# AssafSinger94/dino-tracker

Hardware: AMD Instinct MI355X
Metric: query-points*frames/s (higher is better)
Workload: dtype mixed: fp16 ViT operands (one per value), f16 conv operands in Delta-DINO, f16 candidates + f32 deciders in the tracker; f32 accumulate; 1 GPU; 854x480x90 synthetic video (model res 854x476, 67x121 tokens, C=384), 1024 grid queries; 1 video(s) per step over 1 GPU(s); features=vit, mode=single, track_method=mfma, anchor_pairs=92091, correlation_maps_per_video=8380350, rccl_ranks=1, parallelism=video-parallel x1

## Files before the change

dino_tracker_amd/_lib.py:

```python
from __future__ import annotations

import ctypes
import os

_HERE = os.path.dirname(os.path.abspath(__file__))
LIB_PATH = os.path.join(_HERE, "csrc", "libdtk.so")

c_int, c_float, c_void_p, c_size_t = ctypes.c_int, ctypes.c_float, ctypes.c_void_p, ctypes.c_size_t


class Geom(ctypes.Structure):
    _fields_ = [("T", ctypes.c_int32), ("C", ctypes.c_int32), ("ph", ctypes.c_int32), ("pw", ctypes.c_int32),
                ("video_h", ctypes.c_int32), ("video_w", ctypes.c_int32), ("patch", ctypes.c_int32),
                ("stride", ctypes.c_int32), ("radius", ctypes.c_float)]

    @property
    def HW(self) -> int:
        return self.ph * self.pw


def make_geom(T: int, C: int, video_h: int, video_w: int, patch: int = 14, stride: int = 7, radius: float = 35.0) -> Geom:
    ph = 1 + (video_h - patch) // stride
    pw = 1 + (video_w - patch) // stride
    return Geom(T, C, ph, pw, video_h, video_w, patch, stride, radius)
# ... 62 lines not shown
                [(n, ctypes.c_int64) for n in ("in_stride", "in2_stride", "out_stride", "res_stride", "mul_stride", "gate_stride")])


class RaftModel(ctypes.Structure):
    _fields_ = [("conv", RaftConvDesc * RAFT_NUM_CONVS)]


class TrackStats(ctypes.Structure):
    _fields_ = [("sources", ctypes.c_int32), ("whole_map_tier", ctypes.c_int32), ("exact_tier", ctypes.c_int32),
                ("syncs", ctypes.c_int32)]

    def as_dict(self):
        return {k: int(getattr(self, k)) for k, _ in self._fields_}


SIGNATURES = {
    "dtk_version": (c_int, []),
    "dtk_last_error": (ctypes.c_char_p, []),
    "dtk_profile_enable": (c_int, [c_int]),
    "dtk_profile_collect": (c_int, []),
    "dtk_profile_name": (ctypes.c_char_p, [c_int]),
    "dtk_profile_ms": (ctypes.c_double, [c_int]),
    "dtk_profile_launches": (ctypes.c_longlong, [c_int]),
    "dtk_pack_features": (c_int, [c_void_p, c_void_p, c_void_p, c_int, c_int, c_int, c_void_p]),
    "dtk_unpack_features": (c_int, [c_void_p, c_void_p, c_int, c_int, c_int, c_void_p]),
    "dtk_feature_norms": (c_int, [c_void_p, c_void_p, c_int, c_int, c_int, c_void_p]),
    "dtk_vit_workspace_bytes": (c_size_t, [ctypes.POINTER(VitModel), c_int, c_int, c_int]),
    "dtk_vit_forward": (c_int, [ctypes.POINTER(VitModel), c_void_p, c_int, c_int, c_int, c_void_p, c_void_p, c_void_p,
                                c_void_p, c_size_t, c_void_p]),
    "dtk_vit_attention": (c_int, [c_void_p, c_void_p, c_void_p, c_void_p, c_int, c_int, c_int, c_int, c_int, c_void_p]),
    "dtk_vit_attention_split": (c_int, [c_void_p] * 8 + [c_int, c_int, c_int, c_int, c_int, c_void_p]),
    "dtk_vit_gemm": (c_int, [ctypes.POINTER(VitGemmArgs), c_void_p]),
    "dtk_vit_gemm_split": (c_int, [ctypes.POINTER(VitGemmArgs), c_void_p]),
    "dtk_delta_dino_packed_floats": (c_size_t, [c_int, c_int]),
    "dtk_delta_dino_pack": (c_int, [c_int, c_int, c_void_p, c_void_p, c_void_p, c_void_p, c_void_p, c_void_p, c_float,
                                    c_void_p, c_void_p]),
    "dtk_delta_dino_workspace_bytes": (c_size_t, [ctypes.POINTER(Geom)]),
    "dtk_delta_dino_refine": (c_int, [ctypes.POINTER(Geom), c_void_p, c_void_p, ctypes.POINTER(c_void_p), c_void_p,
                                      c_void_p, c_int, c_int, c_void_p, c_size_t, c_void_p]),
    "dtk_delta_dino_refine_mode": (c_int, [ctypes.POINTER(Geom), c_void_p, c_void_p, ctypes.POINTER(c_void_p), c_void_p,
                                           c_void_p, c_int, c_int, c_int, c_void_p, c_size_t, c_void_p]),
    "dtk_sample_points": (c_int, [ctypes.POINTER(Geom), c_void_p, c_void_p, c_void_p, c_void_p, c_void_p, c_int, c_void_p]),
    "dtk_sample_grid": (c_int, [c_void_p, c_int, c_int, c_int, c_int, c_void_p, c_void_p, c_int, c_void_p]),
    "dtk_normalized_conv2d": (c_int, [c_void_p, c_void_p, c_void_p, c_void_p, c_int, c_int, c_int, c_int, c_int, c_int,
                                      c_void_p]),
    "dtk_corr_maps": (c_int, [ctypes.POINTER(Geom), c_void_p, c_void_p, c_void_p, c_void_p, c_void_p, c_void_p, c_void_p,
                              c_int, c_int, c_void_p]),
    "dtk_head_prepare": (c_int, [c_void_p, c_void_p, c_void_p, c_void_p, c_void_p, c_void_p]),
    "dtk_head_forward": (c_int, [ctypes.POINTER(Geom), c_void_p, c_void_p, c_void_p, c_int, c_int, c_void_p]),
    "dtk_head_forward_train": (c_int, [ctypes.POINTER(Geom), c_void_p, c_void_p, c_void_p, c_void_p, c_int, c_int, c_void_p]),
    "dtk_conv_split_weight_halves": (c_size_t, [c_int, c_int]),
    "dtk_conv_split_pack": (c_int, [c_void_p, c_int, c_int, c_int, c_void_p, c_void_p, c_void_p]),
    "dtk_conv_split_input": (c_int, [c_void_p, c_int, c_int, c_int, c_int, c_int, c_void_p, c_void_p, c_void_p, c_void_p]),
    "dtk_conv_split_run": (c_int, [c_void_p, c_void_p, c_void_p, c_void_p, c_void_p, c_int, c_int, c_int, c_int, c_int, c_int,
                                   c_int, c_int, c_void_p]),
    "dtk_conv_split_output": (c_int, [c_void_p, c_int, c_int, c_int, c_int, c_int, c_int, c_void_p, c_void_p, c_void_p]),
    "dtk_conv_wgrad_split_workspace_bytes": (c_size_t, [c_int, c_int, c_int, c_int, c_int, c_int]),
    "dtk_conv_wgrad_split": (c_int, [c_void_p, c_void_p, c_void_p, c_int, c_int, c_int, c_int, c_int, c_int, c_int, c_void_p,
                                     c_int, c_void_p, c_size_t, c_void_p]),
    "dtk_gemm_nt_f32_indexed": (c_int, [c_void_p, c_void_p, c_void_p, c_int, c_int, c_int, ctypes.c_int64, ctypes.c_int64,
                                        ctypes.c_int64, c_int, ctypes.c_int64, ctypes.c_int64, ctypes.c_int64, c_int, c_int,
                                        c_void_p, c_void_p, c_void_p, c_void_p, c_void_p]),
    "dtk_contrastive_workspace_bytes": (c_size_t, [c_int, c_int, c_int, c_int]),
    "dtk_contrastive_forward": (c_int, [c_void_p, c_void_p, c_void_p, ctypes.c_float, c_int, c_int, c_int, c_int, c_int, c_void_p,
                                        c_void_p, c_void_p, c_void_p, c_void_p, c_void_p]),
    "dtk_contrastive_backward": (c_int, [c_void_p, c_void_p, c_void_p, ctypes.c_float, c_int, c_int, c_int, c_int, c_int, c_void_p,
# ... 150 lines not shown
```

dino_tracker_amd/csrc/vit.hip:

```cpp
#include <stdlib.h>
#include "common.h"
#include "vit_attention4.h"
#include "vit_attention6.h"
#include "vit_gemm_common.h"
#include "vit_rowwise.h"
#include "vit_patch_embed.h"
#include "vit_gemm_tiled.h"
#include "vit_gemm_ws.h"
#include "vit_gemm_ws_ln.h"
#include "vit_gemm_wide.h"
#include "vit_split.h"

namespace {

constexpr int VIT_FRAME_BATCH = 90;

struct VitPlan {
    int S, Sp, FB;
    size_t x, xn, q, k, vt, ao, hid, delta, total;
    bool split;
    size_t xn_lo, q_lo, k_lo, vt_lo, ao_lo, hid_lo;
};

inline bool vit_layer_split(const dtk_vit_layer& L) { return L.qkv_w_lo != nullptr; }
// ... 40 lines not shown
    } else {
        const unsigned grid = attn::attention_grid(FH, S, 128 * attn::A6_NQ, &QB);
        DTK_LAUNCH("vit_attention", (attn::attention6_kernel<T, 0>), dim3(grid), dim3(256), 0, st, q, k, vt, o, S, Sp, heads, D,
                   FH, QB);
    }
    return DTK_OK;
}
template <typename T>
int attention_split_launch(const T* q, const T* q_lo, const T* k, const T* k_lo, const T* vt, const T* vt_lo, T* o, T* o_lo, int frames,
                           int heads, int S, int Sp, hipStream_t st) {
    const int nqb = dtk_cdiv(Sp, 128);
    DTK_LAUNCH("vit_attention_split", attention_split_kernel<T>, dim3((unsigned)(frames * heads * nqb)), dim3(256), 0, st, q, q_lo, k, k_lo,
               vt, vt_lo, o, o_lo, S, Sp, heads, nqb);
    return DTK_OK;
}

struct GemmPath {
    bool tiled;
    bool ws;
    bool wide;
    bool ws_v1;
    bool wide_v1;
    bool fc2_ln;
    bool proj_ln;
};
inline GemmPath gemm_path(int D, int f) {
    const bool tiled = (f & DTK_VIT_TILED_GEMMS) != 0, ws = !tiled && D == WS_K, wide_v1 = (f & DTK_VIT_GEMM_WIDE_V1) != 0;
    static_assert(WS_K == WD_N, "fc2 of the weight-stationary width is gemm_wide_delta_kernel's shape");
    const bool ws_v1 = (f & DTK_VIT_GEMM_WS_V1) != 0, fc2_ln = ws && !wide_v1 && !(f & DTK_VIT_NO_LN_FUSION);
    return {tiled, ws, !tiled && D % W2_N == 0, ws_v1, wide_v1, fc2_ln, fc2_ln && !ws_v1};
}
inline GemmPath gemm_path(const dtk_vit_model* m) { return gemm_path(m->D, m->flags); }

template <typename T, int EPI>
int launch_gemm(const char* name, const GemmPath& path, const T* A, const T* W, long long rows, int N, int K, const GemmEpi<T>& e,
                hipStream_t st) {
    if constexpr (EPI != EPI_F32) {
        const bool ws_fits = EPI != EPI_QKV || e.S >= WS_ROWS || rows <= e.S;
        if constexpr (EPI == EPI_DELTA) {
            if (path.ws && K == WS_K && N == WS_K && e.ln_out) {
                const auto gr = gemm_ws_ln_grid(rows);
                DTK_LAUNCH(name, (gemm_ws_ln_kernel<T>), gr.first, dim3(256), 0, st, A, W, rows, e, gr.second);
                return DTK_OK;
            }
        }
        if (path.ws && K == WS_K && ws_fits) {
            const auto gr = gemm_ws_grid(N, rows);
            if (path.ws_v1)
                DTK_LAUNCH(name, (gemm_ws_kernel<T, EPI, 0>), gr.first, dim3(256), 0, st, A, W, rows, N, e, gr.second);
            else if (N % 64 != 0 || DTK_DBG(e.no_store, 128))
                DTK_LAUNCH(name, (gemm_ws_kernel<T, EPI, 3, false>), gr.first, dim3(256), 0, st, A, W, rows, N, e, gr.second);
            else
                DTK_LAUNCH(name, (gemm_ws_kernel<T, EPI>), gr.first, dim3(256), 0, st, A, W, rows, N, e, gr.second);
            return DTK_OK;
        }
        if (path.ws && EPI == EPI_DELTA) {
            const dim3 grid(dtk_cdiv(rows, WD_M));
            if (path.wide_v1)
                DTK_LAUNCH(name, (gemm_wide_delta_kernel<T, false>), grid, dim3(512), 0, st, A, W, rows, K, e);
            else if (e.ln_out)
                DTK_LAUNCH(name, (gemm_wide_delta_kernel<T, true, true>), grid, dim3(512), 0, st, A, W, rows, K, e);
            else
                DTK_LAUNCH(name, (gemm_wide_delta_kernel<T, true>), grid, dim3(512), 0, st, A, W, rows, K, e);
            return DTK_OK;
        }
        if (path.wide) {
            const dim3 grid(gemm_wide_grid(N, rows));
            if (path.wide_v1)
                DTK_LAUNCH(name, (gemm_wide_kernel<T, EPI, false>), grid, dim3(512), 0, st, A, W, rows, N, K, e);
            else
                DTK_LAUNCH(name, (gemm_wide_kernel<T, EPI, true>), grid, dim3(512), 0, st, A, W, rows, N, K, e);
            return DTK_OK;
        }
    }
    DTK_LAUNCH(name, (gemm_tiled_kernel<T, EPI>), dim3(gemm_grid(N, rows)), dim3(256), 0, st, A, W, rows, N, K, e);
// ... 327 lines not shown
                                 int Sp, int operand_type, void* stream) {
    DTK_REQUIRE(q && k && vt && out, "dtk_vit_attention: null pointer");
    DTK_REQUIRE(frames > 0 && heads > 0 && S > 0 && Sp >= S && Sp % 64 == 0, "dtk_vit_attention: bad sizes (Sp %% 64 == 0, Sp >= S)");
    const bool v4 = (operand_type & DTK_OPERAND_ATTENTION_V4) != 0;
    operand_type &= ~DTK_OPERAND_ATTENTION_V4;
    DTK_REQUIRE(operand_type == DTK_OPERAND_F16 || operand_type == DTK_OPERAND_BF16, "dtk_vit_attention: operand_type");
    return with_operand_type(operand_type == DTK_OPERAND_BF16, [&](auto t) {
        typedef decltype(t) T;
        return attention_launch(reinterpret_cast<const T*>(q), reinterpret_cast<const T*>(k), reinterpret_cast<const T*>(vt),
                                reinterpret_cast<T*>(out), S, Sp, heads, heads * VIT_D_HEAD, frames * heads, v4, dtk_stream(stream));
    });
}

extern "C" int dtk_vit_attention_split(const void* q_hi, const void* q_lo, const void* k_hi, const void* k_lo, const void* vt_hi,
                                       const void* vt_lo, void* out_hi, void* out_lo, int frames, int heads, int S, int Sp,
                                       int operand_type, void* stream) {
    DTK_REQUIRE(q_hi && q_lo && k_hi && k_lo && vt_hi && vt_lo && out_hi && out_lo, "dtk_vit_attention_split: null pointer");
    DTK_REQUIRE(frames > 0 && heads > 0 && S > 0 && Sp >= S && Sp % 64 == 0, "dtk_vit_attention_split: bad sizes (Sp %% 64 == 0, Sp >= S)");
    DTK_REQUIRE(operand_type == DTK_OPERAND_F16 || operand_type == DTK_OPERAND_BF16, "dtk_vit_attention_split: operand_type");
    return with_operand_type(operand_type == DTK_OPERAND_BF16, [&](auto t) {
        typedef decltype(t) T;
        return attention_split_launch<T>((const T*)q_hi, (const T*)q_lo, (const T*)k_hi, (const T*)k_lo, (const T*)vt_hi, (const T*)vt_lo,
                                         (T*)out_hi, (T*)out_lo, frames, heads, S, Sp, dtk_stream(stream));
    });
}

extern "C" int dtk_vit_gemm(const dtk_vit_gemm_args* g, void* stream) {
    if (const int rc = vit_gemm_check(g, "dtk_vit_gemm", false)) return rc;
    return with_operand_type(g->operand_type == DTK_OPERAND_BF16, [&](auto t) {
        return run_gemm<decltype(t)>(*g, gemm_path(g->D, g->flags), vit_gemm_hidden(g), dtk_stream(stream));
    });
}

extern "C" int dtk_vit_gemm_split(const dtk_vit_gemm_args* g, void* stream) {
    if (const int rc = vit_gemm_check(g, "dtk_vit_gemm_split", true)) return rc;
    DTK_REQUIRE(!g->ln_out, "dtk_vit_gemm_split: the split blocks have their own LayerNorm");
    return with_operand_type(g->operand_type == DTK_OPERAND_BF16, [&](auto t) {
        return run_gemm_split<decltype(t)>(*g, gemm_path(g->D, g->flags), vit_gemm_hidden(g), dtk_stream(stream));
    });
}
```

dino_tracker_amd/csrc/vit_gemm_ws.h:

```cpp
#pragma once
#include <type_traits>
#include <utility>
#include "vit_gemm_common.h"

namespace {

constexpr int WS_KS = 24, WS_K = 16 * WS_KS, WS_ROWS = 32, WS_COLS = 256;
constexpr int WS_TILE_BYTES = WS_ROWS * WS_K * 2;
constexpr int WS_LQ = WS_KS / 4;
constexpr int WS_PITCH = 144;
constexpr int WS_UNIT_BYTES = WS_ROWS * WS_PITCH;

template <class F, int... I>
__device__ __forceinline__ void ws_for_each(F&& f, std::integer_sequence<int, I...>) { (f(std::integral_constant<int, I>{}), ...); }
template <int N, class F>
__device__ __forceinline__ void ws_for_each(F&& f) { ws_for_each(f, std::make_integer_sequence<int, N>{}); }

template <typename T, int EPI, int V2M = 3, bool HC = (V2M == 3)>
__global__ __launch_bounds__(256) void gemm_ws_kernel(const T* __restrict__ A, const T* __restrict__ Wt,
                                                      long long M, int N, GemmEpi<T> e, int tiles_per_chunk) {
    typedef typename Vec<T>::t8 T8;
    typedef typename Vec<T>::t4 T4;
    (void)sizeof(T8); (void)sizeof(T4);
    constexpr bool V2 = (V2M & 1) != 0;
    constexpr bool V2D = (V2M & 2) != 0;
    static_assert(!HC || V2M == 3, "the hand-cut step is built on the AGPR weights and the descriptor LDS-DMA");
    operand_mode<T>();
    __shared__ __attribute__((aligned(1024))) unsigned char toks[3][WS_TILE_BYTES];
    __shared__ __attribute__((aligned(16))) unsigned char stage[4][2][WS_UNIT_BYTES];
    __shared__ __attribute__((aligned(16))) float s_bias[4][64], s_gamma[4][64];
    const int tid = threadIdx.x, lane = tid & 63;
    const int w = __builtin_amdgcn_readfirstlane(tid >> 6);
    const int j = lane & 31, h = lane >> 5;
    const int n0 = blockIdx.x * WS_COLS + w * 64;
    const long long total_tiles = (M + WS_ROWS - 1) / WS_ROWS;
    const long long tile0 = (long long)blockIdx.y * tiles_per_chunk;
    if (tile0 >= total_tiles) return;
    const int NT = (int)((total_tiles - tile0) < tiles_per_chunk ? (total_tiles - tile0) : tiles_per_chunk);
    const int nl = (j & 3) + 4 * (j >> 3) + 16 * ((j >> 2) & 1);
    T8 wf[2][WS_KS];
#pragma unroll
    for (int t = 0; t < 2; ++t) {
        const int row = min(n0 + t * 32 + nl, N - 1);
        const T* wp = Wt + (size_t)row * WS_K + h * 8;
#pragma unroll
        for (int ks = 0; ks < WS_KS; ++ks) {
            if (V2) asm volatile("global_load_dwordx4 %0, %1, off" : "=a"(wf[t][ks]) : "v"(wp + ks * 16) : "memory");
            else wf[t][ks] = *reinterpret_cast<const T8*>(wp + ks * 16);
        }
    }
    if (V2) {
        asm volatile("s_waitcnt vmcnt(0)" ::: "memory");
#pragma unroll
        for (int t = 0; t < 2; ++t)
#pragma unroll
            for (int ks = 0; ks < WS_KS; ++ks) asm volatile("" : "+a"(wf[t][ks]));
    }
    if constexpr (!HC) {
        const int n = min(n0 + lane, N - 1);
        s_bias[w][lane] = e.bias ? e.bias[n] : 0.f;
        s_gamma[w][lane] = (EPI == EPI_DELTA) ? e.gamma[n] : 1.f;
    }
    const int which = (EPI == EPI_QKV) ? min(n0, N - 1) / e.D : 0;
    const int head = (EPI == EPI_QKV) ? (min(n0, N - 1) - which * e.D) >> 6 : 0;
    const float qsc = (EPI == EPI_QKV && which == 0) ? e.qscale : 1.f;
    long long m_ep = tile0 * WS_ROWS + j;
    int f_ep = 0, s_ep = 0;
    if (EPI == EPI_QKV) { f_ep = (int)(m_ep / e.S); s_ep = (int)(m_ep - (long long)f_ep * e.S); }
    const unsigned lds_base = (unsigned)(size_t)&toks[0][0];
    const int l_tt = lane & 3, l_pp = lane >> 2;
    const dtk_u4 srd = dtk_make_srd(A + tile0 * WS_ROWS * WS_K);
    unsigned a_voff[2], a_voff_last[2];
    const int last_rows = (int)(M - (total_tiles - 1) * WS_ROWS);
#pragma unroll
    for (int gg = 0; gg < 2; ++gg) {
        const int g = 2 * w + gg;
        a_voff[gg] = (unsigned)(((4 * g + l_tt) * WS_K + ((l_pp - g) & 15) * 8) * 2);
        a_voff_last[gg] = (unsigned)((min(4 * g + l_tt, last_rows - 1) * WS_K + ((l_pp - g) & 15) * 8) * 2);
    }
    const unsigned a_dst = __builtin_amdgcn_readfirstlane(lds_base + (2 * w) * 3 * 1024);
    auto issue = [&](int n, int buf) {
        if (V2D) {
            const unsigned toff = __builtin_amdgcn_readfirstlane((unsigned)n * (unsigned)WS_TILE_BYTES);
            const unsigned dst = __builtin_amdgcn_readfirstlane(a_dst + (unsigned)buf * (unsigned)WS_TILE_BYTES);
            const bool last = tile0 + n == total_tiles - 1;
            const unsigned v0 = last ? a_voff_last[0] : a_voff[0], v1 = last ? a_voff_last[1] : a_voff[1];
            dtk_buffer_lds16<0>(srd, toff, v0, dst);
            dtk_buffer_lds16<1024>(srd, toff + 256u, v0, dst);
            dtk_buffer_lds16<2048>(srd, toff + 512u, v0, dst);
// ... 17 lines not shown
    for (int k8 = 0; k8 < 8; ++k8)
        frag_off[k8] = (unsigned)((j >> 2) * 3 * 1024 + ((((2 * k8 + h + (j >> 2)) & 15) * 4 + (j & 3)) * 16));
    float amax = 0.f;
    unsigned dbg_sink = 0;
    auto dbg_fold = [&](const auto& val) {
        unsigned b[sizeof(val) / 4];
        __builtin_memcpy(b, &val, sizeof(val));
#pragma unroll
        for (unsigned i = 0; i < sizeof(val) / 4; ++i) dbg_sink |= b[i];
    };
    if constexpr (HC) {
        typedef std::integral_constant<bool, true> Yes;
        typedef std::integral_constant<bool, false> No;
        if (n0 >= N) {
            issue(0, 0);
            issue(min(1, NT - 1), 1);
            dtk_vm_wait<WS_LQ>();
            __syncthreads();
            int b0 = 0;
            for (int n = 0; n + 1 < NT; n += 2) {
                const int b1 = b0 == 2 ? 0 : b0 + 1, b2 = b1 == 2 ? 0 : b1 + 1;
                issue(min(n + 2, NT - 1), b2);
                dtk_vm_wait<WS_LQ>();
                __syncthreads();
                issue(min(n + 3, NT - 1), b0);
                dtk_vm_wait<WS_LQ>();
                __syncthreads();
                b0 = b2;
            }
            dtk_vm_wait<0>();
            return;
        }
        float bia[2][16], gam[2][16];
#pragma unroll
        for (int t = 0; t < 2; ++t)
#pragma unroll
            for (int r = 0; r < 16; ++r) {
                const int nf = n0 + 32 * t + 16 * h + r;
                bia[t][r] = e.bias ? e.bias[nf] : 0.f;
                gam[t][r] = (EPI == EPI_DELTA) ? e.gamma[nf] : 1.f;
            }
        const bool dbg_nost = DTK_DBG(e.no_store, 3) || DTK_DBG(e.no_store, 32);
        const bool dbg_noar = DTK_DBG(e.no_store, 64);
        auto run = [&](auto vt_tag) {
            constexpr bool VT = decltype(vt_tag)::value;
            constexpr bool STG = EPI != EPI_GELU && !VT;
            const long long mt0 = tile0 * WS_ROWS;
            T* op = nullptr;
            T* up = nullptr;
            int s0 = 0;
            unsigned cross = 0;
            if constexpr (EPI == EPI_GELU) op = e.out + (mt0 + j) * N + n0 + 16 * h;
            if constexpr (EPI == EPI_DELTA) up = e.delta + mt0 * N + n0;
            if constexpr (EPI == EPI_QKV) {
                const int f0 = (int)(mt0 / e.S);
                s0 = (int)(mt0 - (long long)f0 * e.S);
                if (VT) {
                    up = e.vt + (((size_t)f0 * e.heads + head) * 64) * e.Sp + s0;
                    cross = (unsigned)(e.heads * 64 * e.Sp - e.S);
                } else {
                    up = (which == 0 ? e.q : e.k) + (((size_t)f0 * e.heads + head) * e.Sp + s0) * 64;
                    cross = (unsigned)((e.heads * e.Sp - e.S) * 64);
                }
            }
            const size_t out_step = (size_t)WS_ROWS * N;
            unsigned char* const sw = &stage[w][0][0] + j * WS_PITCH + 32 * h;
            const unsigned char* const sr = &stage[w][0][0] + (lane >> 3) * WS_PITCH + (lane & 7) * 16;
            auto next_tile = [&]() {
                if constexpr (EPI == EPI_GELU) op += out_step;
                if constexpr (EPI == EPI_DELTA) up += out_step;
                if constexpr (EPI == EPI_QKV) {
                    s0 += WS_ROWS;
                    up += VT ? WS_ROWS : WS_ROWS * 64;
                    if (s0 >= e.S) { s0 -= e.S; up += cross; }
                }
            };
            auto st16 = [&](T* p, unsigned off, dtk_u4 val, bool ok) {
                if (!dbg_nost) { if (ok) *reinterpret_cast<dtk_u4*>(p + off) = val; }
                else dbg_fold(val);
            };
            float v[8];
            f2 sx[4], uu[4], pp[4];
            T8 o;
            dtk_u4 fv[4];
            unsigned voff = 0;
            constexpr float GC[9] = {1.112979639e-10f, -1.065557687e-08f, 4.510875158e-07f, -1.125288873e-05f, 1.868377149e-04f,
                                     -2.217123518e-03f, 1.963194646e-02f, -1.326889843e-01f, 7.978046536e-01f};
            auto flush_reads = [&]() {
                ws_for_each<4>([&](auto p_tag) {
                    constexpr int p = decltype(p_tag)::value;
                    fv[p] = *reinterpret_cast<const dtk_u4*>(sr + 8 * p * WS_PITCH);
                });
            };
            auto flush_store = [&](auto pred_tag, auto p_tag, int valid) {
                constexpr int p = decltype(p_tag)::value;
                const int row = 8 * p + (lane >> 3);
                const bool ok = decltype(pred_tag)::value ? row < valid : true;
                if constexpr (EPI == EPI_DELTA) st16(up, (unsigned)(row * N + (lane & 7) * 8), fv[p], ok);
                else st16(up, (unsigned)(row * 64 + (lane & 7) * 8) + (s0 + row >= e.S ? cross : 0u), fv[p], ok);
            };
            auto slot = [&](auto pred_tag, auto fl_tag, const f16v (&acc)[2], auto s_tag, int valid) {
                constexpr bool PRED = decltype(pred_tag)::value, FL = decltype(fl_tag)::value;
                constexpr int s = decltype(s_tag)::value;
                const bool ok = PRED ? j < valid : true;
                if constexpr (EPI == EPI_GELU) {
                    constexpr int u = s / 12, ph = s % 12, t = u >> 1, hv = u & 1;
                    if (ph < 2) {
#pragma unroll
                        for (int r = 4 * ph; r < 4 * ph + 4; ++r) v[r] = acc[t][8 * hv + r] + bia[t][8 * hv + r];
                        if (IsF16<T>::value) {
#pragma unroll
                            for (int r = 4 * ph; r < 4 * ph + 4; r += 2) amax = fmaxf(fmaxf(amax, v[r]), v[r + 1]);
                        }
                    }
                    if (dbg_noar) {
                        if (ph == 9) {
#pragma unroll
                            for (int r = 0; r < 8; ++r) o[r] = (T)v[r];
                        }
                    } else if (ph == 2) {
                        const f2 c = {4.25f, 4.25f};
#pragma unroll
                        for (int q = 0; q < 4; ++q) sx[q] = __builtin_elementwise_min(__builtin_elementwise_max(f2{v[2 * q], v[2 * q + 1]}, -c), c);
#pragma unroll
                        for (int q = 0; q < 4; ++q) uu[q] = sx[q] * sx[q];
                    } else if (ph >= 3 && ph <= 6) {
#pragma unroll
                        for (int l = 2 * (ph - 3); l < 2 * (ph - 3) + 2; ++l)
#pragma unroll
                            for (int q = 0; q < 4; ++q)
                                pp[q] = __builtin_elementwise_fma(l == 0 ? f2{GC[0], GC[0]} : pp[q], uu[q], f2{GC[l + 1], GC[l + 1]});
                    } else if (ph == 7) {
                        const f2 one = {1.f, 1.f};
#pragma unroll
                        for (int q = 0; q < 4; ++q) pp[q] = __builtin_elementwise_min(__builtin_elementwise_max(sx[q] * pp[q], -one), one);
                    } else if (ph == 8) {
#pragma unroll
                        for (int q = 0; q < 4; ++q) {
                            const f2 hx = f2{v[2 * q], v[2 * q + 1]} * f2{0.5f, 0.5f};
                            uu[q] = __builtin_elementwise_fma(hx, pp[q], hx);
                        }
                    } else if (ph == 9) {
#pragma unroll
                        for (int q = 0; q < 4; ++q) { o[2 * q] = (T)uu[q][0]; o[2 * q + 1] = (T)uu[q][1]; }
                    }
                    if (ph == 10) {
                        st16(op, (unsigned)(32 * t + 8 * hv), __builtin_bit_cast(dtk_u4, o), ok);
                    }
                } else if constexpr (STG) {
                    if constexpr (FL && s == 0) flush_reads();
                    if constexpr (FL && s >= 1 && s <= 4) flush_store(No{}, std::integral_constant<int, s - 1>{}, WS_ROWS);
                    constexpr int u = s / 12, ph = s % 12, t = u >> 1, hv = u & 1;
                    if (ph & 1) {
                        if (ph < 9) {
                            constexpr int r0 = (ph - 1) & 7, r1 = ph & 7;
                            const float v0 = acc[t][8 * hv + r0] + bia[t][8 * hv + r0], v1 = acc[t][8 * hv + r1] + bia[t][8 * hv + r1];
                            if (EPI == EPI_QKV && IsF16<T>::value && !dbg_noar) amax = amax2(amax, v0 * qsc, v1 * qsc);
                            if (dbg_noar) { o[r0] = (T)v0; o[r1] = (T)v1; }
                            else if (EPI == EPI_DELTA) { o[r0] = (T)(v0 * gam[t][8 * hv + r0]); o[r1] = (T)(v1 * gam[t][8 * hv + r1]); }
                            else { o[r0] = (T)(v0 * qsc); o[r1] = (T)(v1 * qsc); }
                        } else if (ph == 9) {
                            *reinterpret_cast<T8*>(sw + 64 * t + 16 * hv) = o;
                        }
                    }
                } else {
                    if (s == 0) voff = (unsigned)(16 * h * e.Sp + j) + (s0 + j >= e.S ? cross : 0u);
                    if (s < 32) {
                        constexpr int u = (s & 31) / 8, r = s % 8, t = u >> 1, hv = u & 1;
                        v[r] = acc[t][8 * hv + r] + bia[t][8 * hv + r];
                        if (IsF16<T>::value && (r & 1) && !dbg_noar) amax = amax2(amax, v[r - 1] * qsc, v[r] * qsc);
                        const T val = (T)v[r];
                        T* const p = up + (size_t)(32 * t + 8 * hv + r) * e.Sp;
                        if (!dbg_nost) { if (ok) p[voff] = val; }
                        else dbg_fold(typename Vec<T>::t2{val, val});
                    }
                }
            };
            auto tail_epi = [&](const f16v (&acc)[2], int valid) {
                ws_for_each<2 * WS_KS>([&](auto s_tag) { slot(Yes{}, No{}, acc, s_tag, valid); });
                if (!STG) next_tile();
            };
            auto tail_flush = [&](int valid) {
                if constexpr (STG) {
                    flush_reads();
                    ws_for_each<4>([&](auto p_tag) { flush_store(Yes{}, p_tag, valid); });
                    next_tile();
                }
            };
            auto step = [&](auto prev_tag, auto fl_tag, int buf, f16v (&accN)[2], const f16v (&accP)[2]) {
                constexpr bool PREV = decltype(prev_tag)::value, FL = decltype(fl_tag)::value;
                const unsigned char* base = &toks[0][0] + buf * WS_TILE_BYTES;
                const f16v zero16 = {0.f, 0.f, 0.f, 0.f, 0.f, 0.f, 0.f, 0.f, 0.f, 0.f, 0.f, 0.f, 0.f, 0.f, 0.f, 0.f};
                T8 b[3];
                b[0] = *reinterpret_cast<const T8*>(base + frag_off[0]);
                b[1] = *reinterpret_cast<const T8*>(base + frag_off[1]);
                ws_for_each<2 * WS_KS>([&](auto s_tag) {
                    constexpr int ks = decltype(s_tag)::value / 2, t = decltype(s_tag)::value % 2;
                    if constexpr (t == 0 && ks + 2 < WS_KS)
                        b[(ks + 2) % 3] = *reinterpret_cast<const T8*>(base + frag_off[(ks + 2) & 7] + ((ks + 2) >> 3) * 1024);
                    accN[t] = mfma32(wf[t][ks], b[ks % 3], ks == 0 ? zero16 : accN[t]);
                    if constexpr (PREV) {
                        __builtin_amdgcn_sched_barrier(0);
                        slot(No{}, fl_tag, accP, s_tag, WS_ROWS);
                        __builtin_amdgcn_sched_barrier(0);
                    }
                });
                if (STG ? FL : PREV) next_tile();
            };
            f16v accA[2], accB[2];
            issue(0, 0);
            issue(min(1, NT - 1), 1);
            dtk_vm_wait<WS_LQ>();
            __syncthreads();
            int n = 0, b0 = 0;
            auto pair = [&](auto first_tag) {
                constexpr bool FIRST = decltype(first_tag)::value;
                const int b1 = b0 == 2 ? 0 : b0 + 1, b2 = b1 == 2 ? 0 : b1 + 1;
                issue(min(n + 2, NT - 1), b2);
                if (FIRST) step(No{}, No{}, b0, accA, accB);
                else step(Yes{}, Yes{}, b0, accA, accB);
                dtk_vm_wait<WS_LQ>();
                __syncthreads();
                issue(min(n + 3, NT - 1), b0);
                if (FIRST) step(Yes{}, No{}, b1, accB, accA);
                else step(Yes{}, Yes{}, b1, accB, accA);
                dtk_vm_wait<WS_LQ>();
                __syncthreads();
                b0 = b2;
                n += 2;
            };
            if (NT >= 2) pair(Yes{});
            while (n + 1 < NT) pair(No{});
            const long long left = M - (tile0 + NT - 1) * WS_ROWS;
            const int valid = left < WS_ROWS ? (int)left : WS_ROWS;
            const bool odd = n < NT;
            if (odd) {
                if (n > 0) step(Yes{}, Yes{}, b0, accA, accB);
                else step(No{}, No{}, b0, accA, accB);
            }
            if (NT > 1) tail_flush(WS_ROWS);
            const f16v accL[2] = {odd ? accA[0] : accB[0], odd ? accA[1] : accB[1]};
            tail_epi(accL, valid);
            tail_flush(valid);
        };
        if constexpr (EPI == EPI_QKV) {
            if (which == 2) run(Yes{});
            else run(No{});
        } else {
            run(No{});
        }
        if (DTK_DBG(e.no_store, 32) && dbg_sink == 0x9e3779b9u) amax = 65504.f;
        amax_report<T, EPI>(amax, e.ovf);
        dtk_vm_wait<0>();
        return;
    }
    auto epi8 = [&](const f16v (&acc)[2], int t, int hv) {
        const int fl = 32 * t + 16 * h + 8 * hv;
        const int nb = n0 + fl;
        const float4 b0 = *reinterpret_cast<const float4*>(&s_bias[w][fl]), b1 = *reinterpret_cast<const float4*>(&s_bias[w][fl + 4]);
        float v[8];
#pragma unroll
        for (int r = 0; r < 8; ++r) v[r] = acc[t][8 * hv + r];
        v[0] += b0.x; v[1] += b0.y; v[2] += b0.z; v[3] += b0.w;
        v[4] += b1.x; v[5] += b1.y; v[6] += b1.z; v[7] += b1.w;
        const bool ok = m_ep < M && nb < N && !DTK_DBG(e.no_store, 3);
        if (IsF16<T>::value && (EPI == EPI_QKV || EPI == EPI_GELU)) {
#pragma unroll
            for (int r = 0; r < 8; r += 2) {
                if (EPI == EPI_GELU) amax = fmaxf(fmaxf(amax, v[r]), v[r + 1]);
                else if (!DTK_DBG(e.no_store, 64)) amax = amax2(amax, v[r] * qsc, v[r + 1] * qsc);
            }
        }
        if (EPI == EPI_GELU) {
            T8 o;
#pragma unroll
// ... 139 lines not shown
```

include/dtk.h:

```cpp
#ifndef DTK_H_
#define DTK_H_

#include <stddef.h>
#include <stdint.h>

#ifdef __cplusplus
extern "C" {
#endif

#define DTK_OK 0
#define DTK_E_INVALID (-1)
#define DTK_E_HIP (-2)
#define DTK_E_WORKSPACE (-3)

typedef struct dtk_geom {
    int32_t T;
    int32_t C;
    int32_t ph, pw;
    int32_t video_h, video_w;
    int32_t patch, stride;
    float radius;
} dtk_geom;

#define DTK_HEAD_HIDDEN 16
// ... 67 lines not shown
int dtk_vit_forward(const dtk_vit_model* m, const float* frames, int nframes, int video_h, int video_w,
                    float* tokens_out, float* feat_out, float* qkv_out, void* workspace, size_t workspace_bytes,
                    void* stream);

int dtk_vit_attention(const void* q, const void* k, const void* vt, void* out, int frames, int heads, int S, int Sp,
                      int operand_type, void* stream);
int dtk_vit_attention_split(const void* q_hi, const void* q_lo, const void* k_hi, const void* k_lo, const void* vt_hi,
                            const void* vt_lo, void* out_hi, void* out_lo, int frames, int heads, int S, int Sp, int operand_type,
                            void* stream);

#define DTK_VIT_GEMM_QKV 0
#define DTK_VIT_GEMM_QKV_FACET 1
#define DTK_VIT_GEMM_PROJ 2
#define DTK_VIT_GEMM_FC1 3
#define DTK_VIT_GEMM_FC2 4
#define DTK_VIT_GEMM_FC1_SWIGLU 5
#define DTK_VIT_GEMM_FC2_SWIGLU 6
typedef struct dtk_vit_gemm_args {
    int32_t role, D, flags, operand_type;
    int64_t rows;
    int32_t S, Sp;
    float ln_eps, w_scale;
    const void *a, *a_lo, *w, *w_lo;
    const float *bias, *gamma;
    void *q, *k, *vt, *q_lo, *k_lo, *vt_lo;
    void *out, *out_lo;
    float *out_f32, *x, *ln_x;
    const float *ln_w, *ln_b;
    void* ln_out;
    int32_t* ovf;
} dtk_vit_gemm_args;
int dtk_vit_gemm(const dtk_vit_gemm_args* g, void* stream);
int dtk_vit_gemm_split(const dtk_vit_gemm_args* g, void* stream);

size_t dtk_delta_dino_packed_floats(int layer, int C);
int dtk_delta_dino_pack(int layer, int C, const float* w, const float* bias, const float* bn_w, const float* bn_b,
                        const float* bn_mean, const float* bn_var, float eps, float* packed, void* stream);
size_t dtk_delta_dino_workspace_bytes(const dtk_geom* g);
int dtk_delta_dino_refine(const dtk_geom* g, const float* video, const float* dino, const float* const* packed,
                          float* out, float* norms, int t0, int nframes, void* workspace, size_t workspace_bytes,
                          void* stream);
#define DTK_DD_SPLIT 0
#define DTK_DD_FP16 1
#define DTK_DD_FP16_V1 2
int dtk_delta_dino_refine_mode(const dtk_geom* g, const float* video, const float* dino, const float* const* packed,
                               float* out, float* norms, int t0, int nframes, int operands, void* workspace,
                               size_t workspace_bytes, void* stream);

int dtk_sample_points(const dtk_geom* g, const float* feat, const float* xy, const int32_t* t_idx,
                      const int32_t* out_row, float* out, int B, void* stream);

int dtk_sample_grid(const float* feat, int T, int C, int ph, int pw, const float* pts, float* out, int B, void* stream);

int dtk_head_prepare(const float* w1, const float* b1, const float* w2, const float* b2, float* head, void* stream);

int dtk_head_forward(const dtk_geom* g, const float* head, const float* maps, float* out_xy, int B, int normalized,
                     void* stream);

int dtk_head_forward_train(const dtk_geom* g, const float* head, const float* maps, float* out_xy, float* stats, int B,
                           int normalized, void* stream);
int dtk_head_backward(const dtk_geom* g, const float* head, const float* maps, const float* stats, const float* grad_out,
                      float* dmaps, float* dhead_partial, int B, int normalized, void* stream);

size_t dtk_conv_split_weight_halves(int Cin, int Cout);
int dtk_conv_split_pack(const float* w, int Cin, int Cout, int flip_transpose, void* Wh, void* Wl, void* stream);
int dtk_conv_split_input(const float* x, int N, int C, int H, int W, int border, const float* scale, void* hi, void* lo,
// ... 338 lines not shown
```

Baseline: 528,500 query-points*frames/s.

## Widen weight-stationary fc1/qkv GEMM waves to 96 columns with per-group chunk plan

Adds an RT=3 variant of the weight-stationary GEMM in which each wave holds 96 output columns of weights (partly in AGPRs, partly in VGPRs) instead of 64. A workgroup then covers 384 columns, so each streamed token tile is reused across more MFMAs. A new launch plan splits the grid into column groups with their own tiles-per-chunk, giving the V group of qkv a tuned share of workgroups. QKV output is staged through a larger LDS buffer for coalesced stores, and GELU bias now comes from LDS. The risks are higher register pressure, lower occupancy and a more complex epilogue schedule.

```diff
diff --git a/dino_tracker_amd/_lib.py b/dino_tracker_amd/_lib.py
--- a/dino_tracker_amd/_lib.py
+++ b/dino_tracker_amd/_lib.py
@@ -118,6 +118,8 @@
     "dtk_vit_attention_split": (c_int, [c_void_p] * 8 + [c_int, c_int, c_int, c_int, c_int, c_void_p]),
     "dtk_vit_gemm": (c_int, [ctypes.POINTER(VitGemmArgs), c_void_p]),
     "dtk_vit_gemm_split": (c_int, [ctypes.POINTER(VitGemmArgs), c_void_p]),
+    "dtk_vit_gemm_ws_plan": (c_int, [c_int, c_int, c_int, ctypes.c_int64, c_int, ctypes.POINTER(c_int), ctypes.POINTER(c_int),
+                                     ctypes.POINTER(c_int)]),
     "dtk_delta_dino_packed_floats": (c_size_t, [c_int, c_int]),
     "dtk_delta_dino_pack": (c_int, [c_int, c_int, c_void_p, c_void_p, c_void_p, c_void_p, c_void_p, c_void_p, c_float,
                                     c_void_p, c_void_p]),
diff --git a/dino_tracker_amd/csrc/vit.hip b/dino_tracker_amd/csrc/vit.hip
--- a/dino_tracker_amd/csrc/vit.hip
+++ b/dino_tracker_amd/csrc/vit.hip
@@ -96,15 +96,27 @@
 }
 inline GemmPath gemm_path(const dtk_vit_model* m) { return gemm_path(m->D, m->flags); }
 
+inline bool gemm_ws_fits(int epi, long long rows, int S) { return epi != EPI_QKV || S >= WS_ROWS || rows <= S; }
+inline bool gemm_ws96_runs(const GemmPath& path, int epi, long long rows, int N, int K, int S, int no_store) {
+    return gemm_ws96_role(epi) && path.ws && K == WS_K && gemm_ws_fits(epi, rows, S) && !path.ws_v1 && gemm_ws96_fits(N) && !DTK_DBG(no_store, 128);
+}
+
 template <typename T, int EPI>
 int launch_gemm(const char* name, const GemmPath& path, const T* A, const T* W, long long rows, int N, int K, const GemmEpi<T>& e,
                 hipStream_t st) {
     if constexpr (EPI != EPI_F32) {
-        const bool ws_fits = EPI != EPI_QKV || e.S >= WS_ROWS || rows <= e.S;
+        const bool ws_fits = gemm_ws_fits(EPI, rows, e.S);
         if constexpr (EPI == EPI_DELTA) {
             if (path.ws && K == WS_K && N == WS_K && e.ln_out) {
                 const auto gr = gemm_ws_ln_grid(rows);
                 DTK_LAUNCH(name, (gemm_ws_ln_kernel<T>), gr.first, dim3(256), 0, st, A, W, rows, e, gr.second);
+                return DTK_OK;
+            }
+        }
+        if constexpr (gemm_ws96_role(EPI)) {
+            if (gemm_ws96_runs(path, EPI, rows, N, K, e.S, e.no_store)) {
+                const Ws96Plan plan = gemm_ws96_plan(N, rows);
+                DTK_LAUNCH(name, (gemm_ws_kernel<T, EPI, 3, true, 3>), gemm_ws96_grid(plan), dim3(256), 0, st, A, W, rows, N, e, plan);
                 return DTK_OK;
             }
         }
@@ -498,6 +510,20 @@
     });
 }
 
+extern "C" int dtk_vit_gemm_ws_plan(int role, int D, int flags, int64_t rows, int S, int32_t* chunks, int32_t* tpc, int32_t* last) {
+    if (!chunks || !tpc || !last || rows <= 0 || (role != DTK_VIT_GEMM_FC1 && role != DTK_VIT_GEMM_QKV)) return 0;
+    const int epi = role == DTK_VIT_GEMM_FC1 ? EPI_GELU : EPI_QKV, N = role == DTK_VIT_GEMM_FC1 ? 4 * D : 3 * D;
+    if (!gemm_ws96_runs(gemm_path(D, flags), epi, rows, N, D, S, 0)) return 0;
+    const Ws96Plan p = gemm_ws96_plan(N, rows);
+    const long long tiles = dtk_cdiv(rows, WS_ROWS);
+    for (int g = 0; g < p.groups; ++g) {
+        chunks[g] = p.chunks[g];
+        tpc[g] = p.tpc[g];
+        last[g] = (int32_t)(tiles - (long long)(p.chunks[g] - 1) * p.tpc[g]);
+    }
+    return p.groups;
+}
+
 extern "C" int dtk_vit_gemm_split(const dtk_vit_gemm_args* g, void* stream) {
     if (const int rc = vit_gemm_check(g, "dtk_vit_gemm_split", true)) return rc;
     DTK_REQUIRE(!g->ln_out, "dtk_vit_gemm_split: the split blocks have their own LayerNorm");
diff --git a/dino_tracker_amd/csrc/vit_gemm_ws.h b/dino_tracker_amd/csrc/vit_gemm_ws.h
--- a/dino_tracker_amd/csrc/vit_gemm_ws.h
+++ b/dino_tracker_amd/csrc/vit_gemm_ws.h
@@ -16,45 +16,108 @@
 template <int N, class F>
 __device__ __forceinline__ void ws_for_each(F&& f) { ws_for_each(f, std::make_integer_sequence<int, N>{}); }
 
-template <typename T, int EPI, int V2M = 3, bool HC = (V2M == 3)>
+constexpr int WS96_COLS = 384, WS96_MAX_GROUPS = 4, WS96_WGS = 256;
+constexpr int WS96_PITCH = WS96_COLS * 2 + 16;
+constexpr int WS96_STAGE_BYTES = WS_ROWS * WS96_PITCH;
+constexpr int WS96_VT_SHARE = 92;
+constexpr int WS96_MAX_TPC = 65536;
+struct Ws96Plan {
+    int groups;
+    int chunks[WS96_MAX_GROUPS];
+    int tpc[WS96_MAX_GROUPS];
+};
+inline Ws96Plan gemm_ws96_plan(int N, long long rows) {
+    Ws96Plan p = {};
+    p.groups = N / WS96_COLS;
+    const long long tiles = (rows + WS_ROWS - 1) / WS_ROWS;
+    int vt_share = WS96_VT_SHARE;
+#ifdef DTK_WS96_SWEEP
+    if (const char* sv = getenv("DTK_WS96_VT_SHARE")) vt_share = atoi(sv);
+#endif
+    for (int g = 0; g < p.groups; ++g) {
+        const int share = p.groups != 3 ? WS96_WGS / p.groups : g == 2 ? vt_share : (WS96_WGS - vt_share) / 2;
+        long long tpc = (tiles + share - 1) / share;
+        if (tpc < 1) tpc = 1;
+        if (tpc > WS96_MAX_TPC) tpc = WS96_MAX_TPC;
+        p.tpc[g] = (int)tpc;
+        p.chunks[g] = (int)((tiles + tpc - 1) / tpc);
+    }
+    return p;
+}
+constexpr bool gemm_ws96_role(int epi) { return epi == EPI_GELU || epi == EPI_QKV; }
+inline bool gemm_ws96_fits(int N) { return N % WS96_COLS == 0 && N / WS96_COLS >= 1 && N / WS96_COLS <= WS96_MAX_GROUPS; }
+inline dim3 gemm_ws96_grid(const Ws96Plan& p) {
+    unsigned n = 0;
+    for (int g = 0; g < p.groups; ++g) n += (unsigned)p.chunks[g];
+    return dim3(n);
+}
+struct WsWhere {
+    unsigned colgroup;
+    int tpc;
+    unsigned chunk;
+};
+template <int RT> struct WsArg { typedef int type; };
+template <> struct WsArg<3> { typedef Ws96Plan type; };
+__device__ __forceinline__ WsWhere ws_where(int tiles_per_chunk) {
+    return {blockIdx.x, tiles_per_chunk, blockIdx.y};
+}
+__device__ __forceinline__ WsWhere ws_where(const Ws96Plan& plan) {
+    int c = blockIdx.x, g = 0, tpc = plan.tpc[0], first = 0;
+#pragma unroll
+    for (int i = 0; i + 1 < WS96_MAX_GROUPS; ++i) {
+        first += plan.chunks[i];
+        if (i + 1 < plan.groups && (int)blockIdx.x >= first) { g = i + 1; c = (int)blockIdx.x - first; tpc = plan.tpc[i + 1]; }
+    }
+    return {(unsigned)g, tpc, (unsigned)c};
+}
+
+template <typename T, int EPI, int V2M = 3, bool HC = (V2M == 3), int RT = 2>
 __global__ __launch_bounds__(256) void gemm_ws_kernel(const T* __restrict__ A, const T* __restrict__ Wt,
-                                                      long long M, int N, GemmEpi<T> e, int tiles_per_chunk) {
+                                                      long long M, int N, GemmEpi<T> e, typename WsArg<RT>::type where) {
     typedef typename Vec<T>::t8 T8;
     typedef typename Vec<T>::t4 T4;
     (void)sizeof(T8); (void)sizeof(T4);
     constexpr bool V2 = (V2M & 1) != 0;
     constexpr bool V2D = (V2M & 2) != 0;
     static_assert(!HC || V2M == 3, "the hand-cut step is built on the AGPR weights and the descriptor LDS-DMA");
+    static_assert(RT == 2 || (RT == 3 && HC && (EPI == EPI_GELU || EPI == EPI_QKV)), "96 features per wave: the hand-cut fc1 and qkv steps only");
+    constexpr int WCOLS = 32 * RT;
+    constexpr int AGPR_FRAGS = RT == 2 ? 2 * WS_KS : 60;
     operand_mode<T>();
     __shared__ __attribute__((aligned(1024))) unsigned char toks[3][WS_TILE_BYTES];
     __shared__ __attribute__((aligned(16))) unsigned char stage[4][2][WS_UNIT_BYTES];
-    __shared__ __attribute__((aligned(16))) float s_bias[4][64], s_gamma[4][64];
+    constexpr bool STG3 = RT == 3 && EPI == EPI_QKV;
+    __shared__ __attribute__((aligned(16))) unsigned char stage3[STG3 ? 2 : 1][STG3 ? WS96_STAGE_BYTES : 16];
+    __shared__ __attribute__((aligned(16))) float s_bias[4][WCOLS], s_gamma[4][64];
     const int tid = threadIdx.x, lane = tid & 63;
     const int w = __builtin_amdgcn_readfirstlane(tid >> 6);
     const int j = lane & 31, h = lane >> 5;
-    const int n0 = blockIdx.x * WS_COLS + w * 64;
+    const WsWhere wh = ws_where(where);
+    const int tiles_per_chunk = wh.tpc;
+    const int n0 = wh.colgroup * (4 * WCOLS) + w * WCOLS;
     const long long total_tiles = (M + WS_ROWS - 1) / WS_ROWS;
-    const long long tile0 = (long long)blockIdx.y * tiles_per_chunk;
+    const long long tile0 = (long long)wh.chunk * tiles_per_chunk;
     if (tile0 >= total_tiles) return;
     const int NT = (int)((total_tiles - tile0) < tiles_per_chunk ? (total_tiles - tile0) : tiles_per_chunk);
     const int nl = (j & 3) + 4 * (j >> 3) + 16 * ((j >> 2) & 1);
-    T8 wf[2][WS_KS];
-#pragma unroll
-    for (int t = 0; t < 2; ++t) {
+    T8 wf[RT][WS_KS];
+#pragma unroll
+    for (int t = 0; t < RT; ++t) {
         const int row = min(n0 + t * 32 + nl, N - 1);
         const T* wp = Wt + (size_t)row * WS_K + h * 8;
 #pragma unroll
         for (int ks = 0; ks < WS_KS; ++ks) {
-            if (V2) asm volatile("global_load_dwordx4 %0, %1, off" : "=a"(wf[t][ks]) : "v"(wp + ks * 16) : "memory");
+            if (V2 && t * WS_KS + ks < AGPR_FRAGS) asm volatile("global_load_dwordx4 %0, %1, off" : "=a"(wf[t][ks]) : "v"(wp + ks * 16) : "memory");
             else wf[t][ks] = *reinterpret_cast<const T8*>(wp + ks * 16);
         }
     }
     if (V2) {
         asm volatile("s_waitcnt vmcnt(0)" ::: "memory");
 #pragma unroll
-        for (int t = 0; t < 2; ++t)
-#pragma unroll
-            for (int ks = 0; ks < WS_KS; ++ks) asm volatile("" : "+a"(wf[t][ks]));
+        for (int t = 0; t < RT; ++t)
+#pragma unroll
+            for (int ks = 0; ks < WS_KS; ++ks)
+                if (t * WS_KS + ks < AGPR_FRAGS) asm volatile("" : "+a"(wf[t][ks]));
     }
     if constexpr (!HC) {
         const int n = min(n0 + lane, N - 1);
@@ -138,14 +201,19 @@
             return;
         }
         float bia[2][16], gam[2][16];
-#pragma unroll
-        for (int t = 0; t < 2; ++t)
-#pragma unroll
-            for (int r = 0; r < 16; ++r) {
-                const int nf = n0 + 32 * t + 16 * h + r;
-                bia[t][r] = e.bias ? e.bias[nf] : 0.f;
-                gam[t][r] = (EPI == EPI_DELTA) ? e.gamma[nf] : 1.f;
-            }
+        if constexpr (RT == 2) {
+#pragma unroll
+            for (int t = 0; t < 2; ++t)
+#pragma unroll
+                for (int r = 0; r < 16; ++r) {
+                    const int nf = n0 + 32 * t + 16 * h + r;
+                    bia[t][r] = e.bias ? e.bias[nf] : 0.f;
+                    gam[t][r] = (EPI == EPI_DELTA) ? e.gamma[nf] : 1.f;
+                }
+        } else {
+            (void)bia; (void)gam;
+            for (int i = lane; i < WCOLS; i += 64) s_bias[w][i] = e.bias ? e.bias[n0 + i] : 0.f;
+        }
         const bool dbg_nost = DTK_DBG(e.no_store, 3) || DTK_DBG(e.no_store, 32);
         const bool dbg_noar = DTK_DBG(e.no_store, 64);
         auto run = [&](auto vt_tag) {
@@ -168,6 +236,10 @@
                     up = (which == 0 ? e.q : e.k) + (((size_t)f0 * e.heads + head) * e.Sp + s0) * 64;
                     cross = (unsigned)((e.heads * e.Sp - e.S) * 64);
                 }
+                if constexpr (RT == 3) {
+                    if (VT) up = e.vt + ((size_t)f0 * e.heads * 64 + (n0 - which * e.D)) * e.Sp + s0;
+                    else up = (which == 0 ? e.q : e.k) + ((size_t)f0 * e.heads * e.Sp + s0) * 64;
+                }
             }
             const size_t out_step = (size_t)WS_ROWS * N;
             unsigned char* const sw = &stage[w][0][0] + j * WS_PITCH + 32 * h;
@@ -188,28 +260,88 @@
             float v[8];
             f2 sx[4], uu[4], pp[4];
             T8 o;
-            dtk_u4 fv[4];
+            constexpr int NFL = STG3 ? 6 : 4;
+            dtk_u4 fv[NFL];
             unsigned voff = 0;
+            unsigned sto = 0, flo = 0;
+            unsigned char* const sw3 = STG3 ? &stage3[0][0] + j * WS96_PITCH + (w * WCOLS + 16 * h) * 2 : nullptr;
+            const unsigned char* const sr3 = STG3 ? &stage3[0][0] + (tid >> 3) * WS96_PITCH + (lane & 7) * 16 : nullptr;
             constexpr float GC[9] = {1.112979639e-10f, -1.065557687e-08f, 4.510875158e-07f, -1.125288873e-05f, 1.868377149e-04f,
                                      -2.217123518e-03f, 1.963194646e-02f, -1.326889843e-01f, 7.978046536e-01f};
             auto flush_reads = [&]() {
-                ws_for_each<4>([&](auto p_tag) {
+                ws_for_each<NFL>([&](auto p_tag) {
                     constexpr int p = decltype(p_tag)::value;
-                    fv[p] = *reinterpret_cast<const dtk_u4*>(sr + 8 * p * WS_PITCH);
+                    if constexpr (STG3) fv[p] = *reinterpret_cast<const dtk_u4*>(sr3 + flo + 128 * p);
+                    else fv[p] = *reinterpret_cast<const dtk_u4*>(sr + 8 * p * WS_PITCH);
                 });
             };
             auto flush_store = [&](auto pred_tag, auto p_tag, int valid) {
                 constexpr int p = decltype(p_tag)::value;
+                if constexpr (STG3) {
+                    const int row3 = tid >> 3;
+                    const bool ok3 = decltype(pred_tag)::value ? row3 < valid : true;
+                    st16(up, (unsigned)(row3 * 64 + (lane & 7) * 8 + p * e.Sp * 64) + (s0 + row3 >= e.S ? cross : 0u), fv[p], ok3);
+                    return;
+                }
                 const int row = 8 * p + (lane >> 3);
                 const bool ok = decltype(pred_tag)::value ? row < valid : true;
                 if constexpr (EPI == EPI_DELTA) st16(up, (unsigned)(row * N + (lane & 7) * 8), fv[p], ok);
                 else st16(up, (unsigned)(row * 64 + (lane & 7) * 8) + (s0 + row >= e.S ? cross : 0u), fv[p], ok);
             };
-            auto slot = [&](auto pred_tag, auto fl_tag, const f16v (&acc)[2], auto s_tag, int valid) {
+            float4 bi0, bi1, bj0, bj1;
+            auto slot = [&](auto pred_tag, auto fl_tag, const f16v (&acc)[RT], auto s_tag, int valid) {
                 constexpr bool PRED = decltype(pred_tag)::value, FL = decltype(fl_tag)::value;
                 constexpr int s = decltype(s_tag)::value;
                 const bool ok = PRED ? j < valid : true;
-                if constexpr (EPI == EPI_GELU) {
+                if constexpr (EPI == EPI_GELU && RT == 3) {
+                    const float* const sb = &s_bias[w][16 * h];
+                    constexpr int u = s / 12, ph = s % 12, t = u >> 1, hv = u & 1;
+                    if (ph == 0) {
+                        bi0 = *reinterpret_cast<const float4*>(sb + 32 * t + 8 * hv);
+                        bi1 = *reinterpret_cast<const float4*>(sb + 32 * t + 8 * hv + 4);
+                    } else if (ph <= 2) {
+                        const float4 bq = ph == 1 ? bi0 : bi1;
+                        const float bb[4] = {bq.x, bq.y, bq.z, bq.w};
+#pragma unroll
+                        for (int r = 4 * (ph - 1); r < 4 * (ph - 1) + 4; ++r) v[r] = acc[t][8 * hv + r] + bb[r & 3];
+                        if (IsF16<T>::value) {
+#pragma unroll
+                            for (int r = 4 * (ph - 1); r < 4 * (ph - 1) + 4; r += 2) amax = fmaxf(fmaxf(amax, v[r]), v[r + 1]);
+                        }
+                    }
+                    if (dbg_noar) {
+                        if (ph == 10) {
+#pragma unroll
+                            for (int r = 0; r < 8; ++r) o[r] = (T)v[r];
+                        }
+                    } else if (ph == 3) {
+                        const f2 c = {4.25f, 4.25f};
+#pragma unroll
+                        for (int q = 0; q < 4; ++q) sx[q] = __builtin_elementwise_min(__builtin_elementwise_max(f2{v[2 * q], v[2 * q + 1]}, -c), c);
+#pragma unroll
+                        for (int q = 0; q < 4; ++q) uu[q] = sx[q] * sx[q];
+                    } else if (ph >= 4 && ph <= 7) {
+#pragma unroll
+                        for (int l = 2 * (ph - 4); l < 2 * (ph - 4) + 2; ++l)
+#pragma unroll
+                            for (int q = 0; q < 4; ++q)
+                                pp[q] = __builtin_elementwise_fma(l == 0 ? f2{GC[0], GC[0]} : pp[q], uu[q], f2{GC[l + 1], GC[l + 1]});
+                    } else if (ph == 8) {
+                        const f2 one = {1.f, 1.f};
+#pragma unroll
+                        for (int q = 0; q < 4; ++q) pp[q] = __builtin_elementwise_min(__builtin_elementwise_max(sx[q] * pp[q], -one), one);
+                    } else if (ph == 9) {
+#pragma unroll
+                        for (int q = 0; q < 4; ++q) {
+                            const f2 hx = f2{v[2 * q], v[2 * q + 1]} * f2{0.5f, 0.5f};
+                            uu[q] = __builtin_elementwise_fma(hx, pp[q], hx);
+                        }
+                    } else if (ph == 10) {
+#pragma unroll
+                        for (int q = 0; q < 4; ++q) { o[2 * q] = (T)uu[q][0]; o[2 * q + 1] = (T)uu[q][1]; }
+                    }
+                    if (ph == 11) st16(op, (unsigned)(32 * t + 8 * hv), __builtin_bit_cast(dtk_u4, o), ok);
+                } else if constexpr (EPI == EPI_GELU) {
                     constexpr int u = s / 12, ph = s % 12, t = u >> 1, hv = u & 1;
                     if (ph < 2) {
 #pragma unroll
@@ -252,6 +384,52 @@
                     }
                     if (ph == 10) {
                         st16(op, (unsigned)(32 * t + 8 * hv), __builtin_bit_cast(dtk_u4, o), ok);
+                    }
+                } else if constexpr (STG3 && STG) {
+                    const float* const sb = &s_bias[w][16 * h];
+                    if constexpr (FL && s == 0) flush_reads();
+                    if constexpr (FL && s >= 1 && s <= NFL) flush_store(No{}, std::integral_constant<int, s - 1>{}, WS_ROWS);
+                    constexpr int u = s / 12, ph = s % 12, t = u >> 1, hv = u & 1;
+                    if constexpr (ph == 0) {
+                        bi0 = *reinterpret_cast<const float4*>(sb + 32 * t + 8 * hv);
+                        bi1 = *reinterpret_cast<const float4*>(sb + 32 * t + 8 * hv + 4);
+                    } else if constexpr ((ph & 1) && ph < 9) {
+                        constexpr int r0 = (ph - 1) & 7, r1 = ph & 7;
+                        const float bb[8] = {bi0.x, bi0.y, bi0.z, bi0.w, bi1.x, bi1.y, bi1.z, bi1.w};
+                        const float v0 = acc[t][8 * hv + r0] + bb[r0], v1 = acc[t][8 * hv + r1] + bb[r1];
+                        if (IsF16<T>::value && !dbg_noar) amax = amax2(amax, v0 * qsc, v1 * qsc);
+                        if (dbg_noar) { o[r0] = (T)v0; o[r1] = (T)v1; }
+                        else { o[r0] = (T)(v0 * qsc); o[r1] = (T)(v1 * qsc); }
+                    } else if constexpr (ph == 9) {
+                        *reinterpret_cast<T8*>(sw3 + sto + 64 * t + 16 * hv) = o;
+                    }
+                } else if constexpr (STG3) {
+                    const float* const sb = &s_bias[w][16 * h];
+                    if constexpr (s == 0) {
+                        voff = (unsigned)(16 * h * e.Sp + j) + (s0 + j >= e.S ? cross : 0u);
+                        bi0 = *reinterpret_cast<const float4*>(sb);
+                        bi1 = *reinterpret_cast<const float4*>(sb + 4);
+                    }
+                    if constexpr (s < 16 * RT) {
+                        constexpr int u = s / 8, r = s % 8, t = u >> 1, hv = u & 1;
+                        if constexpr (r == 3 && u + 1 < 2 * RT) {
+                            constexpr int tn = (u + 1) >> 1, hn = (u + 1) & 1;
+                            if constexpr (u & 1) {
+                                bi0 = *reinterpret_cast<const float4*>(sb + 32 * tn + 8 * hn);
+                                bi1 = *reinterpret_cast<const float4*>(sb + 32 * tn + 8 * hn + 4);
+                            } else {
+                                bj0 = *reinterpret_cast<const float4*>(sb + 32 * tn + 8 * hn);
+                                bj1 = *reinterpret_cast<const float4*>(sb + 32 * tn + 8 * hn + 4);
+                            }
+                        }
+                        const float4 q0 = (u & 1) ? bj0 : bi0, q1 = (u & 1) ? bj1 : bi1;
+                        const float bb[8] = {q0.x, q0.y, q0.z, q0.w, q1.x, q1.y, q1.z, q1.w};
+                        v[r] = acc[t][8 * hv + r] + bb[r];
+                        if (IsF16<T>::value && (r & 1) && !dbg_noar) amax = amax2(amax, v[r - 1] * qsc, v[r] * qsc);
+                        const T val = (T)v[r];
+                        T* const p = up + (size_t)(32 * t + 8 * hv + r) * e.Sp;
+                        if (!dbg_nost) { if (ok) p[voff] = val; }
+                        else dbg_fold(typename Vec<T>::t2{val, val});
                     }
                 } else if constexpr (STG) {
                     if constexpr (FL && s == 0) flush_reads();
@@ -282,26 +460,26 @@
                     }
                 }
             };
-            auto tail_epi = [&](const f16v (&acc)[2], int valid) {
-                ws_for_each<2 * WS_KS>([&](auto s_tag) { slot(Yes{}, No{}, acc, s_tag, valid); });
+            auto tail_epi = [&](const f16v (&acc)[RT], int valid) {
+                ws_for_each<RT * WS_KS>([&](auto s_tag) { slot(Yes{}, No{}, acc, s_tag, valid); });
                 if (!STG) next_tile();
             };
             auto tail_flush = [&](int valid) {
                 if constexpr (STG) {
                     flush_reads();
-                    ws_for_each<4>([&](auto p_tag) { flush_store(Yes{}, p_tag, valid); });
+                    ws_for_each<NFL>([&](auto p_tag) { flush_store(Yes{}, p_tag, valid); });
                     next_tile();
                 }
             };
-            auto step = [&](auto prev_tag, auto fl_tag, int buf, f16v (&accN)[2], const f16v (&accP)[2]) {
+            auto step = [&](auto prev_tag, auto fl_tag, int buf, f16v (&accN)[RT], const f16v (&accP)[RT]) {
                 constexpr bool PREV = decltype(prev_tag)::value, FL = decltype(fl_tag)::value;
                 const unsigned char* base = &toks[0][0] + buf * WS_TILE_BYTES;
                 const f16v zero16 = {0.f, 0.f, 0.f, 0.f, 0.f, 0.f, 0.f, 0.f, 0.f, 0.f, 0.f, 0.f, 0.f, 0.f, 0.f, 0.f};
                 T8 b[3];
                 b[0] = *reinterpret_cast<const T8*>(base + frag_off[0]);
                 b[1] = *reinterpret_cast<const T8*>(base + frag_off[1]);
-                ws_for_each<2 * WS_KS>([&](auto s_tag) {
-                    constexpr int ks = decltype(s_tag)::value / 2, t = decltype(s_tag)::value % 2;
+                ws_for_each<RT * WS_KS>([&](auto s_tag) {
+                    constexpr int ks = decltype(s_tag)::value / RT, t = decltype(s_tag)::value % RT;
                     if constexpr (t == 0 && ks + 2 < WS_KS)
                         b[(ks + 2) % 3] = *reinterpret_cast<const T8*>(base + frag_off[(ks + 2) & 7] + ((ks + 2) >> 3) * 1024);
                     accN[t] = mfma32(wf[t][ks], b[ks % 3], ks == 0 ? zero16 : accN[t]);
@@ -313,7 +491,7 @@
                 });
                 if (STG ? FL : PREV) next_tile();
             };
-            f16v accA[2], accB[2];
+            f16v accA[RT], accB[RT];
             issue(0, 0);
             issue(min(1, NT - 1), 1);
             dtk_vm_wait<WS_LQ>();
@@ -323,11 +501,13 @@
                 constexpr bool FIRST = decltype(first_tag)::value;
                 const int b1 = b0 == 2 ? 0 : b0 + 1, b2 = b1 == 2 ? 0 : b1 + 1;
                 issue(min(n + 2, NT - 1), b2);
+                if constexpr (STG3) { sto = WS96_STAGE_BYTES; flo = 0; }
                 if (FIRST) step(No{}, No{}, b0, accA, accB);
                 else step(Yes{}, Yes{}, b0, accA, accB);
                 dtk_vm_wait<WS_LQ>();
                 __syncthreads();
                 issue(min(n + 3, NT - 1), b0);
+                if constexpr (STG3) { sto = 0; flo = WS96_STAGE_BYTES; }
                 if (FIRST) step(Yes{}, No{}, b1, accB, accA);
                 else step(Yes{}, Yes{}, b1, accB, accA);
                 dtk_vm_wait<WS_LQ>();
@@ -341,12 +521,27 @@
             const int valid = left < WS_ROWS ? (int)left : WS_ROWS;
             const bool odd = n < NT;
             if (odd) {
+                if constexpr (STG3) { sto = WS96_STAGE_BYTES; flo = 0; }
                 if (n > 0) step(Yes{}, Yes{}, b0, accA, accB);
                 else step(No{}, No{}, b0, accA, accB);
             }
+            if constexpr (STG3 && STG) {
+                __syncthreads();
+                flo = odd ? WS96_STAGE_BYTES : 0;
+                sto = odd ? 0 : WS96_STAGE_BYTES;
+            }
             if (NT > 1) tail_flush(WS_ROWS);
-            const f16v accL[2] = {odd ? accA[0] : accB[0], odd ? accA[1] : accB[1]};
-            tail_epi(accL, valid);
+            if constexpr (RT == 2) {
+                const f16v accL[2] = {odd ? accA[0] : accB[0], odd ? accA[1] : accB[1]};
+                tail_epi(accL, valid);
+            } else {
+                const f16v accL[3] = {odd ? accA[0] : accB[0], odd ? accA[1] : accB[1], odd ? accA[2] : accB[2]};
+                tail_epi(accL, valid);
+            }
+            if constexpr (STG3 && STG) {
+                __syncthreads();
+                flo = sto;
+            }
             tail_flush(valid);
         };
         if constexpr (EPI == EPI_QKV) {
diff --git a/include/dtk.h b/include/dtk.h
--- a/include/dtk.h
+++ b/include/dtk.h
@@ -123,6 +123,7 @@
 } dtk_vit_gemm_args;
 int dtk_vit_gemm(const dtk_vit_gemm_args* g, void* stream);
 int dtk_vit_gemm_split(const dtk_vit_gemm_args* g, void* stream);
+int dtk_vit_gemm_ws_plan(int role, int D, int flags, int64_t rows, int S, int32_t* chunks, int32_t* tpc, int32_t* last);
 
 size_t dtk_delta_dino_packed_floats(int layer, int C);
 int dtk_delta_dino_pack(int layer, int C, const float* w, const float* bias, const float* bn_w, const float* bn_b,
```

After: 536,200 query-points*frames/s, median of 6. 1.01x the previous value.
